# iosefa/obia

Measured on AMD Instinct MI355X. Metric: Mpixel/s (SLIC+zonal feats) on 16384²×8-band; achieved HBM GB/s fraction, higher is better.
Workload: dtype f32

## Files before the change

obia_amd/csrc/slic_spatial.hip:

```cpp

#ifdef OBIA_RUN_STATS
__device__ unsigned long long g_run_stats[16];
#define RS_DECL unsigned long long rs_t = clock64(); unsigned rs_c[8] = {0, 0, 0, 0, 0, 0, 0, 0};
#define RS_COUNT(i, v) rs_c[i] += (unsigned)(v);
#define RS_TICK(i) { const unsigned long long rs_n = clock64(); if ((threadIdx.x & 63) == 0) atomicAdd(&g_run_stats[i], rs_n - rs_t); rs_t = rs_n; }
#define RS_FLUSH { for (int rs_i = 1; rs_i < 8; ++rs_i) { unsigned rs_v = rs_c[rs_i]; for (int rs_o = 32; rs_o; rs_o >>= 1) rs_v += __shfl_xor(rs_v, rs_o); \
                   if ((threadIdx.x & 63) == 0) atomicAdd(&g_run_stats[rs_i], (unsigned long long)rs_v); } if ((threadIdx.x & 63) == 0) atomicAdd(&g_run_stats[0], 1ull); }
extern "C" void obia_debug_run_stats(unsigned long long *out, int reset) {
    (void)hipMemcpyFromSymbol(out, HIP_SYMBOL(g_run_stats), sizeof(unsigned long long) * 16);
    if (reset) { unsigned long long z[16] = {0}; (void)hipMemcpyToSymbol(HIP_SYMBOL(g_run_stats), z, sizeof(z)); }
}
#else
#define RS_DECL
#define RS_COUNT(i, v)
#define RS_TICK(i)
#define RS_FLUSH
#endif

constexpr float RUN_REL = 0x1p-19f, RUN_ABS = 0x1p-60f, RUN_W_LO = 0x1p-30f, RUN_W_HI = 0x1p90f;

template <int CP>
__device__ __forceinline__ void slic_spatial_tile(const SlicProblem &P, int gtile, int tile, int l_n, const unsigned *__restrict__ mask4,
                                                  const float *__restrict__ cent, unsigned long long *__restrict__ acc, int RQ,
                                                  unsigned long long *__restrict__ px_counter, int *__restrict__ orphan_flag,
                                                  const int *__restrict__ tl_k, const unsigned *__restrict__ tl_fp) {
    constexpr int RS = CENT_REC + CP;
    constexpr int NW = NT / 64;
    constexpr unsigned INF_BITS = 0x7f800000u;
    __shared__ __attribute__((aligned(16))) float r_hdr[MAXC][CENT_REC];
    __shared__ int r_k[MAXC];
    __shared__ unsigned long long r_acc[MAXC];
    __shared__ unsigned char r_surv[NW][SWEEP_TW / FB][64];
    __shared__ unsigned r_q[NW][128];

    const int tid = threadIdx.x;
    const int wv = __builtin_amdgcn_readfirstlane(tid >> 6);
    const int ty0 = (tile / P.tiles_x) * SWEEP_TH, tx0 = (tile % P.tiles_x) * SWEEP_TW;
    const float w = P.spatial_w;
    RS_DECL
    if (px_counter && tile == 0 && tid == 0) atomicAdd(px_counter, (unsigned long long)P.H * (unsigned long long)P.W);

    int lk = -1;
    if (tid < l_n) lk = tl_k[(size_t)gtile * MAXC + tid];
    const unsigned myc4 = tl_fp[(size_t)gtile * NT + tid];
    if (tid < MAXC) r_acc[tid] = 0ull;
    if (lk >= 0) {
        const float4 *src = reinterpret_cast<const float4 *>(cent + (size_t)lk * RS);
        const float4 a = src[0], b = src[1];
        float4 *dh = reinterpret_cast<float4 *>(&r_hdr[tid][0]);
        dh[0] = a; dh[1] = b;
        r_k[tid] = lk;
    }
    const int nc = l_n;
    __syncthreads();
    RS_TICK(8)

    const int fy0 = ty0 + FB * wv;
    if (fy0 < P.H) {
        const int fy1 = min(fy0 + FB, P.H);
        const int lane = lane_now();
        int cnt[SWEEP_TW / FB];
#pragma unroll
        for (int bxi = 0; bxi < SWEEP_TW / FB; ++bxi) {
            const int fx0 = tx0 + FB * bxi;
            cnt[bxi] = 0;
            if (fx0 >= P.W) continue;
            const int fx1 = min(fx0 + FB, P.W);
            const unsigned c = (myc4 >> (8 * bxi)) & 0xffu;
            unsigned lbb = 0xffffffffu, ubb = INF_BITS;
            bool hit = false;
            if (c != 0xffu) {
                const float4 h0 = *reinterpret_cast<const float4 *>(&r_hdr[c][0]);
                const float2 h1 = *reinterpret_cast<const float2 *>(&r_hdr[c][4]);
                const int y0 = __float_as_int(h0.z), y1 = __float_as_int(h0.w), x0 = __float_as_int(h1.x), x1 = __float_as_int(h1.y);
                if (y0 < fy1 && y1 > fy0 && x0 < fx1 && x1 > fx0) {
                    hit = true;
                    const float cy = h0.x, cx = h0.y;
                    const float ylo = (float)fy0, yhi = (float)(fy1 - 1), xlo = (float)fx0, xhi = (float)(fx1 - 1);
                    const float ry = (cy < ylo) ? ylo : ((cy > yhi) ? yhi : cy), rx = (cx < xlo) ? xlo : ((cx > xhi) ? xhi : cx);
                    const float tyn = cy - ry, txn = cx - rx;
                    lbb = __float_as_uint((tyn * tyn + txn * txn) * w);
                    if (y0 <= fy0 && y1 >= fy1 && x0 <= fx0 && x1 >= fx1) {
                        const float tyf = fmaxf(fabsf(cy - ylo), fabsf(cy - yhi)), txf = fmaxf(fabsf(cx - xlo), fabsf(cx - xhi));
                        ubb = __float_as_uint((tyf * tyf + txf * txf) * w);
                    }
                }
            }
            const unsigned bound = wave_umin(ubb);
            bool surv = hit && lbb <= bound;
            if (bound != INF_BITS) {
                const int la = (int)__builtin_ctzll(__ballot(ubb == bound));
                const int ca = __builtin_amdgcn_readlane((int)c, la);
                const float4 ha = *reinterpret_cast<const float4 *>(&r_hdr[ca][0]);
                const float4 hb = *reinterpret_cast<const float4 *>(&r_hdr[surv ? c : ca][0]);
                const float ylo = (float)fy0, yhi = (float)(fy1 - 1), xlo = (float)fx0, xhi = (float)(fx1 - 1);
                const float ay0 = (ha.x - ylo) * (ha.x - ylo), ay1 = (ha.x - yhi) * (ha.x - yhi), ax0 = (ha.y - xlo) * (ha.y - xlo), ax1 = (ha.y - xhi) * (ha.y - xhi);
                const float by0 = (hb.x - ylo) * (hb.x - ylo), by1 = (hb.x - yhi) * (hb.x - yhi), bx0 = (hb.y - xlo) * (hb.y - xlo), bx1 = (hb.y - xhi) * (hb.y - xhi);
                const float a00 = (ay0 + ax0) * w, a01 = (ay0 + ax1) * w, a10 = (ay1 + ax0) * w, a11 = (ay1 + ax1) * w;
                const float g = fminf(fminf((by0 + bx0) * w - a00, (by0 + bx1) * w - a01), fminf((by1 + bx0) * w - a10, (by1 + bx1) * w - a11));
                const float M = fmaxf(fmaxf(a00, a01), fmaxf(a10, a11));
                if (M < 3.0e38f && g > RUN_REL * M + RUN_ABS * w) surv = false;
            }
            const unsigned long long m = __ballot(surv);
            const unsigned pos = __builtin_amdgcn_mbcnt_hi((unsigned)(m >> 32), __builtin_amdgcn_mbcnt_lo((unsigned)m, 0u));
            if (surv) r_surv[wv][bxi][pos] = (unsigned char)c;
            cnt[bxi] = __popcll(m);
        }
        wave_lds_sync();
        RS_TICK(9)

        const int seg = lane >> 4, y = fy0 + (lane & 15), xa = tx0 + FB * seg;
        const int mycnt = seg == 0 ? cnt[0] : (seg == 1 ? cnt[1] : (seg == 2 ? cnt[2] : cnt[3]));
        const unsigned char *sv = &r_surv[wv][seg][0];
        unsigned rowbits = 0u;
        if (y < P.H && xa < P.W) {
            const int n = min(FB, P.W - xa);
            if ((long long)P.n_valid == (long long)P.H * (long long)P.W) {
                rowbits = 0xffffu >> (FB - n);
            } else {
                const unsigned *mp = mask4 + ((long long)P.m4_off + (long long)(y >> 2) * P.W + xa);
                const int sh = 8 * (y & 3);
#pragma unroll
                for (int i = 0; i < FB; ++i) {
                    const unsigned v = (i < n) ? mp[i] : 0u;
                    rowbits |= (unsigned)(((v >> sh) & 0xffu) != 0u) << i;
                }
            }
        }
        const float fy = (float)y;
        bool orphan = false;
        auto add_run = [&](int k, int a, int b) {
            const unsigned bits = rowbits & (0xffffu >> (FB - 1 - (b - xa))) & (0xffffu << (a - xa)) & 0xffffu;
            if (!bits) return;
            if (k < 0) { orphan = true; return; }
            const unsigned m = __popc(bits);
            const unsigned sx = __popc(bits & 0xaaaau) + 2u * __popc(bits & 0xccccu) + 4u * __popc(bits & 0xf0f0u) + 8u * __popc(bits & 0xff00u) +
                                m * (unsigned)(xa - tx0);
// ... 47 lines not shown
                int m = xl + (int)(gl / (gl + gr) * (float)(len - 1));
                m = max(xl + 1, min(m, xr - 2));
                const int p0 = m - 1, p3 = m + 2;
                const float fp0 = (float)p0, fm = (float)m, fm1 = (float)(m + 1), fp3 = (float)p3;
                float e1p0 = INFINITY, e2p0 = INFINITY, e1p3 = INFINITY, e2p3 = INFINITY, e1m = INFINITY, e1m1 = INFINITY, dump = INFINITY;
                int kp0 = -1, kp3 = -1, km = -1, km1 = -1;
                for (int i = 0; i < mycnt; ++i) {
                    const int c = sv[i];
                    const float4 h0 = *reinterpret_cast<const float4 *>(&r_hdr[c][0]);
                    const float2 h1 = *reinterpret_cast<const float2 *>(&r_hdr[c][4]);
                    const int y0 = __float_as_int(h0.z), y1 = __float_as_int(h0.w), x0 = __float_as_int(h1.x), x1 = __float_as_int(h1.y);
                    if ((unsigned)(y - y0) >= (unsigned)(y1 - y0)) continue;
                    const float ty = h0.x - fy, dy2 = ty * ty;
                    const float t0 = h0.y - fp0, t1 = h0.y - fm, t2 = h0.y - fm1, t3 = h0.y - fp3;
                    take((dy2 + t0 * t0) * w, p0 >= x0 && p0 < x1, c, e1p0, e2p0, kp0);
                    take((dy2 + t1 * t1) * w, m >= x0 && m < x1, c, e1m, dump, km);
                    take((dy2 + t2 * t2) * w, m + 1 >= x0 && m + 1 < x1, c, e1m1, dump, km1);
                    take((dy2 + t3 * t3) * w, p3 >= x0 && p3 < x1, c, e1p3, e2p3, kp3);
                }
                const bool okl = kp0 == k1l && (p0 == xl || margin(d1l, d2l, e1p0, e2p0));
                const bool okr = kp3 == k1r && (p3 == xr || margin(e1p3, e2p3, d1r, d2r));
                bool mdone = false, m1done = false;
                if (okl) { mdone = km == k1l; add_run(k1l, xl, mdone ? m : p0); } else q0 = entry(xl, p0);
                if (okr) { m1done = km1 == k1r; add_run(k1r, m1done ? m + 1 : p3, xr); } else q1 = entry(p3, xr);
                if (!mdone) add_run(km, m, m);
                if (!m1done) add_run(km1, m + 1, m + 1);
            } else {
                q0 = entry(xl, xr);
            }
        }
        int qn = 0;
        {
            const unsigned long long m0 = __ballot(q0 != 0xffffffffu);
            if (q0 != 0xffffffffu) r_q[wv][__builtin_amdgcn_mbcnt_hi((unsigned)(m0 >> 32), __builtin_amdgcn_mbcnt_lo((unsigned)m0, 0u))] = q0;
            qn = __popcll(m0);
            const unsigned long long m1 = __ballot(q1 != 0xffffffffu);
            if (q1 != 0xffffffffu) r_q[wv][qn + __builtin_amdgcn_mbcnt_hi((unsigned)(m1 >> 32), __builtin_amdgcn_mbcnt_lo((unsigned)m1, 0u))] = q1;
            qn += __popcll(m1);
        }
        wave_lds_sync();
        RS_TICK(10)
        RS_COUNT(5, lane == 0 ? qn : 0)
        for (int base = 0; base < qn; base += 4) {
            const int ei = base + (lane >> 4);
            if (ei >= qn) continue;
            const unsigned e = r_q[wv][ei];
            const int xrel = (int)(e & 15u) + (lane & 15);
            if (xrel > (int)((e >> 4) & 15u) || !((e >> (16 + xrel)) & 1u)) continue;
            RS_COUNT(6, 1)
            const int qs = (int)((e >> 12) & 3u), qy = fy0 + (int)((e >> 8) & 15u), qx = tx0 + FB * qs + xrel;
            const int qcnt = qs == 0 ? cnt[0] : (qs == 1 ? cnt[1] : (qs == 2 ? cnt[2] : cnt[3]));
            const unsigned char *qv = &r_surv[wv][qs][0];
            const float fqy = (float)qy, fqx = (float)qx;
            float best = INFINITY;
            int bk = -1;
            for (int i = 0; i < qcnt; ++i) {
                const int c = qv[i];
                const float4 h0 = *reinterpret_cast<const float4 *>(&r_hdr[c][0]);
                const float2 h1 = *reinterpret_cast<const float2 *>(&r_hdr[c][4]);
                const int y0 = __float_as_int(h0.z), y1 = __float_as_int(h0.w), x0 = __float_as_int(h1.x), x1 = __float_as_int(h1.y);
                if (!(qy >= y0 && qy < y1 && qx >= x0 && qx < x1)) continue;
                const float ty = h0.x - fqy, tx = h0.y - fqx;
                const float d = (ty * ty + tx * tx) * w;
                if (d < best) { best = d; bk = c; }
            }
            if (bk < 0) orphan = true;
            else atomicAdd(&r_acc[bk], 1ull | ((unsigned long long)(unsigned)(qy - ty0) << 16) | ((unsigned long long)(unsigned)(qx - tx0) << 40));
        }
        if (__ballot(orphan) && lane == 0) *orphan_flag = 1;
        RS_TICK(11)
        RS_FLUSH
    }
    __syncthreads();
    const int tid_e = wv * 64 + lane_now();
    for (int i = tid_e; i < nc * 3; i += NT) {
        const int slot = i / 3, q = i - slot * 3;
        const unsigned long long pw = r_acc[slot];
        const unsigned long long n = pw & 0xffffull;
        if (n == 0ull) continue;
        const unsigned long long v = q == 0 ? n : (q == 1 ? ((pw >> 16) & 0xffffffull) + n * (unsigned long long)ty0 : (pw >> 40) + n * (unsigned long long)tx0);
        atomicAdd(&acc[(size_t)r_k[slot] * RQ + CP + q], v);
    }
    RS_TICK(12)
}

template <int CP>
__global__ __launch_bounds__(NT) __attribute__((amdgpu_waves_per_eu(LEAN_WAVES, LEAN_WAVES))) void slic_spatial_kernel(OBIA_ASSIGN_PARAMS) {
    constexpr int XG = OBIA_XCD_GROUP;
    const int gtile = tile_base + (((int)(blockIdx.x >> 3) / XG) * 8 + (int)(blockIdx.x & 7)) * XG + (int)(blockIdx.x >> 3) % XG;
    if (gtile >= total_tiles_all) return;
    const int l_n = tl_meta[2 * (size_t)gtile], l_bw = tl_meta[2 * (size_t)gtile + 1], l_req = tl_req[gtile];
    const int prob_i = tiles_per_prob > 0 ? gtile / tiles_per_prob : tile_prob[gtile];
    const SlicProblem P = probs[prob_i];
    const bool listed = l_n >= 0 && l_bw >= 0 && l_req <= (l_bw & 0xffff);
    if (listed && accumulate && !store_labels && !P.direct && P.spatial_w >= RUN_W_LO && P.spatial_w <= RUN_W_HI)
        slic_spatial_tile<CP>(P, gtile, gtile - P.tile_off, l_n, mask4, cent, acc, RQ, px_counter, orphan_flag, tl_k, tl_fp);
    else
        slic_assign_body<CP, true, true, false, false, true, false>(OBIA_ASSIGN_ARGS);
}
```

obia_amd/csrc/slic_sweep.hip:

```cpp
#include "slic.hpp"

#include <type_traits>
#include <hip/hip_ext.h>

#include <cstdlib>

namespace obia {

#ifdef OBIA_STAMP
__device__ unsigned long long g_tl[65536 * 4 * 24];
#define STAMP_DECL unsigned long long st_t = clock64(), st_t0 = st_t, st_r0 = __builtin_amdgcn_s_memrealtime(), st_acc[12] = {0, 0, 0, 0, 0, 0, 0, 0, 0, 0, 0, 0}, st_cnt[6] = {0, 0, 0, 0, 0, 0};
#define STAMP_COUNT(i, v) st_cnt[i] += (v);
#define STAMP(i) { const unsigned long long st_n = clock64(); st_acc[i] += st_n - st_t; st_t = st_n; }
#ifndef OBIA_STAMP_KIND
#define OBIA_STAMP_KIND 0
#endif
#define STAMP_FLUSH if (accumulate && (LEAN ? 1 : 0) == OBIA_STAMP_KIND && (threadIdx.x & 63) == 0 && gtile < 65536) { unsigned long long *st_o = g_tl + ((size_t)gtile * 4 + (threadIdx.x >> 6)) * 24; for (int st_i = 0; st_i < 12; ++st_i) st_o[st_i] = st_acc[st_i]; st_o[12] = st_t0; st_o[13] = clock64(); st_o[14] = st_r0; st_o[15] = __builtin_amdgcn_s_memrealtime(); for (int st_i = 0; st_i < 6; ++st_i) st_o[16 + st_i] = st_cnt[st_i]; }
#else
#define STAMP_DECL
#define STAMP(i)
#define STAMP_COUNT(i, v)
#define STAMP_FLUSH
#endif

// ... 240 lines not shown

__device__ __forceinline__ void wave_lds_sync() {
    asm volatile("" ::: "memory");
    __builtin_amdgcn_wave_barrier();
    asm volatile("" ::: "memory");
}

__device__ __forceinline__ int lane_now() { return (int)__builtin_amdgcn_mbcnt_hi(~0u, __builtin_amdgcn_mbcnt_lo(~0u, 0u)); }

template <int CP>
__device__ __forceinline__ void global_accumulate(unsigned long long *__restrict__ acc, int RQ, int k, unsigned y, unsigned x,
                                                  const float *f, float fs) {
    unsigned long long *a = acc + (size_t)k * RQ;
#pragma unroll
    for (int ch = 0; ch < CP; ++ch) atomicAdd(&a[ch], (unsigned long long)(long long)to_fixed32(f[ch], fs));
    atomicAdd(&a[CP], 1ull);
    atomicAdd(&a[CP + 1], (unsigned long long)y);
    atomicAdd(&a[CP + 2], (unsigned long long)x);
}

__device__ __forceinline__ bool orphan_needs_repeat(int store_labels, int sweep_id) {
    return store_labels == 0 || (store_labels == 1 && sweep_id > 1);
}

template <int CP, bool MASKED, bool IGNORE_COLOR, bool SLICZERO>
__device__ void slow_tile(const SlicProblem &P, int ty0, int tx0, const float *__restrict__ feat,
                          const uint8_t *__restrict__ mask, const float *__restrict__ cent,
                          const int *__restrict__ head, int32_t *__restrict__ labels,
                          unsigned long long *__restrict__ acc, int RQ, int accumulate, int accum_color, int start_label,
                          float fs, int store_labels, int *__restrict__ orphan_flag, int sweep_id, int nch) {
    constexpr int RS = CENT_REC + CP;
    const float w = P.spatial_w;
    for (int i = threadIdx.x; i < SWEEP_TW * SWEEP_TH; i += NT) {
        const int y = ty0 + i / SWEEP_TW, x = tx0 + i % SWEEP_TW;
        if (y >= P.H || x >= P.W) continue;
        const long long pix = P.pix_off + (long long)y * P.W + x;
        if (MASKED && mask[pix] == 0) { labels[pix] = start_label - 1; continue; }
        float f[CP];
#pragma unroll
        for (int ch = 0; ch < CP; ++ch) f[ch] = ch < nch ? feat_at(feat, P, CP, y, x, ch) : 0.0f;
        int by_lo = (y - 2 * P.sy - 2) / P.sy; if (y - 2 * P.sy - 2 < 0) by_lo = 0;
        int by_hi = (y + 2 * P.sy + 2) / P.sy; if (by_hi > P.ncy - 1) by_hi = P.ncy - 1;
        int bx_lo = (x - 2 * P.sx - 2) / P.sx; if (x - 2 * P.sx - 2 < 0) bx_lo = 0;
        int bx_hi = (x + 2 * P.sx + 2) / P.sx; if (bx_hi > P.ncx - 1) bx_hi = P.ncx - 1;
        float best = INFINITY;
        int bk = -1;
        for (int by = by_lo; by <= by_hi; ++by)
            for (int bx = bx_lo; bx <= bx_hi; ++bx)
                for (int cur = head[P.cell_off + by * P.ncx + bx]; cur >= 0; cur = reinterpret_cast<const int *>(cent + (size_t)cur * RS)[6]) {
                    const float *rec = cent + (size_t)cur * RS;
                    const int *irec = reinterpret_cast<const int *>(rec);
                    if (!(y >= irec[2] && y < irec[3] && x >= irec[4] && x < irec[5])) continue;
                    const float tyv = P.sp_y * (rec[0] - (float)y), txv = P.sp_x * (rec[1] - (float)x);
                    const float dy2 = tyv * tyv, dx2 = txv * txv;
                    float d = (dy2 + dx2) * w;
                    if (!IGNORE_COLOR) {
                        float dc = 0.0f;
#pragma unroll
                        for (int ch = 0; ch < CP; ++ch) { const float t = f[ch] - rec[CENT_REC + ch]; dc += t * t; }
                        d += SLICZERO ? dc / rec[7] : dc;
                    }
                    if (d < best || (d == best && cur < bk)) { best = d; bk = cur; }
                }
        int k = bk;
        if (k < 0) {
            if (orphan_needs_repeat(store_labels, sweep_id)) *orphan_flag = 1;
            if (store_labels == 2) {
                const int prev = labels[pix];
                if (prev >= start_label) k = prev - start_label + P.cent_off;
            }
        } else {
            labels[pix] = k - P.cent_off + start_label;
        }
        if (accumulate && k >= 0) {
            if (!accum_color) {
#pragma unroll
                for (int ch = 0; ch < CP; ++ch) f[ch] = 0.0f;
            }
            global_accumulate<CP>(acc, RQ, k, (unsigned)y, (unsigned)x, f, fs);
        }
    }
}

template <int CP, bool MASKED, bool IGNORE_COLOR, bool FIXPT, bool SLICZERO, bool LEAN, bool COLLB, int NCH = CP>
__device__ __forceinline__ void slic_assign_body(
    const SlicProblem *__restrict__ probs, const float *__restrict__ feat, const uint8_t *__restrict__ mask,
    const unsigned *__restrict__ mask4, const float *__restrict__ cent, const int *__restrict__ head,
    int32_t *__restrict__ labels, unsigned long long *__restrict__ acc, int RQ, int accumulate, int store_labels,
    int start_label, float fs, const int *__restrict__ bin_stamp, int *__restrict__ tile_lp,
    int *__restrict__ cache_k, unsigned long long *__restrict__ cache_q, int sweep_id, int use_cache,
    unsigned long long *__restrict__ px_counter, const int *__restrict__ tile_prob, int total_tiles_all,
    int *__restrict__ orphan_flag, int tiles_per_prob, const float *__restrict__ fbox, int tile_base, int nch_arg,
    int *__restrict__ tl_k, unsigned *__restrict__ tl_fp, int *__restrict__ tl_meta, const int *__restrict__ tl_req) {
    const int nch_rt = (NCH < CP) ? NCH : nch_arg;
    constexpr int accum_color = LEAN ? 0 : 1;
#ifdef OBIA_ABL_NOACC
    accumulate = 0;
#endif
#ifndef OBIA_XCD_GROUP
#define OBIA_XCD_GROUP 2
#endif
    constexpr int XG = OBIA_XCD_GROUP;
    const int gtile = tile_base + (((int)(blockIdx.x >> 3) / XG) * 8 + (int)(blockIdx.x & 7)) * XG + (int)(blockIdx.x >> 3) % XG;
    if (gtile >= total_tiles_all) return;
    const int l_n = tl_meta[2 * (size_t)gtile], l_bw = tl_meta[2 * (size_t)gtile + 1], l_req = tl_req[gtile];
    const int l_built = l_bw < 0 ? -1 : (l_bw & 0xffff), l_streak = l_bw < 0 ? 0 : (l_bw >> 16);
    STAMP_DECL
    constexpr int RS = CENT_REC + CP;
    const int prob_i = tiles_per_prob > 0 ? gtile / tiles_per_prob : tile_prob[gtile];
    const SlicProblem P = probs[prob_i];
    const int tile = gtile - P.tile_off;
    constexpr int AQ = LEAN ? 1 : CP + 1;
    constexpr int PWI = LEAN ? 0 : CP;
    constexpr int NPASS = (CP + 7) / 8;

    __shared__ __attribute__((aligned(16))) float s_hdr[MAXC][CENT_REC];
    __shared__ __attribute__((aligned(16))) float s_col[COLLB ? MAXC : 1][COLLB ? CP : 4];
    __shared__ __attribute__((aligned(16))) int s_k[MAXC];
    __shared__ unsigned char s_fls[NT / 64][64];
    __shared__ unsigned long long s_acc[MAXC][AQ];
    constexpr int NF = LEAN ? 1 : CP + 1;
#ifndef OBIA_FOLD_LAYERS
#define OBIA_FOLD_LAYERS 1
#endif
    constexpr int FOLD_LAYERS = LEAN ? 0 : OBIA_FOLD_LAYERS;
    constexpr int FLD = FOLD_LAYERS > 0 ? FOLD_LAYERS : 1;
    __shared__ int s_tf[LEAN ? 1 : NT / 64][FLD][NF][LEAN ? 1 : 65];
    __shared__ int s_tkey[LEAN ? 1 : NT / 64][FLD][LEAN ? 1 : 64];
    __shared__ unsigned s_orph[SWEEP_TH * SWEEP_TW / 32];
    __shared__ int s_cnt, s_uncacheable;
#ifdef OBIA_ABL_LDSPAD
    __shared__ int s_pad[OBIA_ABL_LDSPAD / 4];
    if (start_label == 12345) s_pad[threadIdx.x] = 1;
#endif

    const int tid = threadIdx.x, lane = tid & 63;
    const int wv = __builtin_amdgcn_readfirstlane(tid >> 6);
    const int ty0 = (tile / P.tiles_x) * SWEEP_TH, tx0 = (tile % P.tiles_x) * SWEEP_TW;
    const int ty1 = min(ty0 + SWEEP_TH, P.H), tx1 = min(tx0 + SWEEP_TW, P.W);
    if (P.direct) {
        slow_tile<CP, MASKED, IGNORE_COLOR, SLICZERO>(P, ty0, tx0, feat, mask, cent, head, labels, acc, RQ, accumulate,
                                                      accum_color, start_label, fs, store_labels, orphan_flag, sweep_id, nch_rt);
        return;
    }

    const float w = P.spatial_w;
    const int fy0 = ty0 + FB * wv;
    const int fy0_o = fy0;
    const bool wave_active = fy0 < P.H;
    const int fy1 = min(fy0 + FB, P.H);
    const int fy1_o = fy1;
    const bool want_feat = !IGNORE_COLOR || accum_color;
    v2f f2[LEAN ? 1 : CP][PPT / 2];
    unsigned mbw;
    const bool all_valid = (long long)P.n_valid == (long long)P.H * (long long)P.W;
    auto fetch = [&](int fx0, int yb, int lane_o, bool real) {
#ifdef OBIA_ABL_NOLOAD
        real = false;
#endif
        const int xx = fx0 + (lane_o & 15);
        if (MASKED && !all_valid) {
            const unsigned *mbase = mask4 + ((long long)P.m4_off + (long long)(fy0 >> 2) * P.W + fx0);
            const unsigned moff = (real && (yb < P.H) && (xx < P.W)) ? (unsigned)(lane_o >> 4) * (unsigned)P.W + (unsigned)(lane_o & 15) : 0u;
            mbw = mbase[moff];
        } else {
            mbw = 0x01010101u;
        }
        if (!LEAN && want_feat) {
            const float4 *pb = reinterpret_cast<const float4 *>(feat) +
                               (P.feat_off + ((long long)(fy0 >> 2) * P.XB + (fx0 >> 4)) * ((LEAN ? 0 : CP) * 16));
            const unsigned fob = (real && (yb < P.H) && (xx < P.W))
                                     ? ((unsigned)(lane_o >> 4) * (unsigned)((LEAN ? 0 : CP) * 16 * P.XB) + (unsigned)(lane_o & 15)) * 16u : 0u;
#pragma unroll
            for (int ch = 0; ch < (LEAN ? 1 : CP); ++ch) {
                if (ch >= nch_rt) { f2[ch][0] = splat(0.0f); f2[ch][1] = splat(0.0f); continue; }
                const float4 t = ld_stream_f4(reinterpret_cast<const char *>(pb + ch * 16) + (size_t)fob);
                f2[ch][0] = (v2f){t.x, t.y};
                f2[ch][1] = (v2f){t.z, t.w};
            }
        } else {
#pragma unroll
            for (int ch = 0; ch < (LEAN ? 1 : CP); ++ch) { f2[ch][0] = splat(0.0f); f2[ch][1] = splat(0.0f); }
        }
    };
    auto fetch_first = [&]() {
        const int lane_i = lane_now();
        fetch(tx0, fy0 + PPT * (lane_i >> 4), lane_i, true);
    };
    constexpr int GQ = CP + 3;
    const int tile_id = P.tile_off + tile;
    int by_lo = (ty0 - 2 * P.sy - 2) / P.sy; if (ty0 - 2 * P.sy - 2 < 0) by_lo = 0;
    int by_hi = (ty1 + 2 * P.sy + 1) / P.sy; if (by_hi > P.ncy - 1) by_hi = P.ncy - 1;
    int bx_lo = (tx0 - 2 * P.sx - 2) / P.sx; if (tx0 - 2 * P.sx - 2 < 0) bx_lo = 0;
    int bx_hi = (tx1 + 2 * P.sx + 1) / P.sx; if (bx_hi > P.ncx - 1) bx_hi = P.ncx - 1;
    const int nbw = bx_hi - bx_lo + 1;
    const int nbins = (by_hi - by_lo + 1) * nbw;
    if (FIXPT) {
        const int lp = use_cache ? tile_lp[tile_id] : 0;
        int dirty = lp <= 0;
        if (!dirty)
            for (int bi = tid; bi < nbins; bi += NT)
                dirty |= bin_stamp[P.cell_off + (by_lo + bi / nbw) * P.ncx + bx_lo + bi % nbw] > lp;
        if (!__syncthreads_or(dirty)) {
            if (accumulate) {
                const int *ck = cache_k + (size_t)tile_id * (MAXC + 1);
                const unsigned long long *cq = cache_q + (size_t)tile_id * MAXC * GQ;
                const int ne = ck[0];
                for (int i = tid; i < ne * GQ; i += NT) {
                    const int e = i / GQ, q = i - e * GQ;
                    const int k = ck[1 + e];
                    if (k < 0 || (q < CP && !accum_color)) continue;
                    atomicAdd(&acc[(size_t)k * RQ + q], cq[(size_t)e * GQ + q]);
                }
            }
            return;
        }
        if (px_counter && tid == 0) atomicAdd(&px_counter[tile & 255], (unsigned long long)(ty1 - ty0) * (unsigned long long)(tx1 - tx0));
    } else if (px_counter && tile == 0 && tid == 0) {
        atomicAdd(px_counter, (unsigned long long)P.H * (unsigned long long)P.W);
    }
#ifdef OBIA_NO_LISTS
    constexpr bool USE_LISTS = false;
#else
    constexpr bool USE_LISTS = !COLLB;
#endif
    const bool listed = USE_LISTS && l_n >= 0 && l_req <= l_built;
    unsigned myc4 = 0xffffffffu;
    auto clear_tables = [&]() {
        for (int i = tid; i < MAXC * AQ; i += NT) (&s_acc[0][0])[i] = 0ull;
        for (int i = tid; i < SWEEP_TH * SWEEP_TW / 32; i += NT) s_orph[i] = 0u;
        if (tid == 0) s_uncacheable = 0;
    };
    float4 r0 = make_float4(0.f, 0.f, 0.f, 0.f), r1 = r0, rcol[CP / 4];
#pragma unroll
    for (int q = 0; q < CP / 4; ++q) rcol[q] = r0;
    int nxt = -1;
    auto load_node = [&](int c) {
        const float4 *src = reinterpret_cast<const float4 *>(cent + (size_t)c * RS);
        r0 = src[0]; r1 = src[1];
        if (COLLB) {
#pragma unroll
            for (int q = 0; q < CP / 4; ++q) rcol[q] = src[2 + q];
        }
        nxt = __float_as_int(r1.z);
    };
    auto put_slot = [&](int slot, int k) {
        float4 *dh = reinterpret_cast<float4 *>(&s_hdr[slot][0]);
        dh[0] = r0; dh[1] = make_float4(r1.x, r1.y, __int_as_float(k), r1.w);
        s_k[slot] = k;
        if (COLLB) {
#pragma unroll
            for (int q = 0; q < CP / 4; ++q) *reinterpret_cast<float4 *>(&s_col[slot][4 * q]) = rcol[q];
        }
    };
    int nc;
    if (listed) {
        int lk = -1;
        if (tid < l_n) lk = tl_k[(size_t)gtile * MAXC + tid];
        myc4 = tl_fp[(size_t)gtile * NT + tid];
        clear_tables();
        if (lk >= 0) load_node(lk);
        if (wave_active) fetch_first();
        if (lk >= 0) put_slot(tid, lk);
        nc = l_n;
        __syncthreads();
        STAMP(1)
    } else {
        clear_tables();
        const int streak = (l_n >= 0 && sweep_id - l_built <= 1) ? l_streak + 1 : 0;
        int g = (!USE_LISTS || l_n == -2 || streak >= LIST_GIVE_UP || sweep_id >= 0xffff) ? 0 : LIST_G2;
        bool listable = g > 0;
        for (;;) {
            __syncthreads();
            if (tid < MAXC) s_k[tid] = 0x7fffffff;
            if (tid == 0) s_cnt = 0;
            __syncthreads();
            int gy_lo = (ty0 - 2 * P.sy - 2 - g) / P.sy; if (ty0 - 2 * P.sy - 2 - g < 0) gy_lo = 0;
            int gy_hi = (ty1 + 2 * P.sy + 1 + g) / P.sy; if (gy_hi > P.ncy - 1) gy_hi = P.ncy - 1;
            int gx_lo = (tx0 - 2 * P.sx - 2 - g) / P.sx; if (tx0 - 2 * P.sx - 2 - g < 0) gx_lo = 0;
            int gx_hi = (tx1 + 2 * P.sx + 1 + g) / P.sx; if (gx_hi > P.ncx - 1) gx_hi = P.ncx - 1;
            const int gbw = gx_hi - gx_lo + 1;
            const int gbins = (gy_hi - gy_lo + 1) * gbw;
            for (int bi = tid; bi < gbins; bi += NT) {
                int cur = head[P.cell_off + (gy_lo + bi / gbw) * P.ncx + gx_lo + bi % gbw];
                if (cur >= 0) load_node(cur);
                while (cur >= 0) {
                    const int y0 = __float_as_int(r0.z), y1 = __float_as_int(r0.w);
                    const int x0 = __float_as_int(r1.x), x1 = __float_as_int(r1.y);
                    if (y0 - g < ty1 && y1 + g > ty0 && x0 - g < tx1 && x1 + g > tx0) {
                        const int slot = atomicAdd(&s_cnt, 1);
                        if (slot < MAXC) put_slot(slot, cur);
                    }
                    cur = nxt;
                    if (cur >= 0) load_node(cur);
                }
            }
            __syncthreads();
            nc = s_cnt;
            if (nc > MAXC) {
                if (g > 0) { g = 0; listable = false; continue; }
                if (tid == 0) { tl_meta[2 * (size_t)gtile] = -2; tl_meta[2 * (size_t)gtile + 1] = sweep_id & 0xffff; }
                slow_tile<CP, MASKED, IGNORE_COLOR, SLICZERO>(P, ty0, tx0, feat, mask, cent, head, labels, acc, RQ, accumulate,
                                                              accum_color, start_label, fs, store_labels, orphan_flag, sweep_id, nch_rt);
                return;
            }
            {
                int myk = 0, rk = 0;
                if (tid < nc) {
                    myk = s_k[tid];
#pragma unroll 1
                    for (int i = 0; i < nc; i += 8) {
                        const int4 ka = *reinterpret_cast<const int4 *>(&s_k[i]), kb = *reinterpret_cast<const int4 *>(&s_k[i + 4]);
                        rk += (ka.x < myk) + (ka.y < myk) + (ka.z < myk) + (ka.w < myk) + (kb.x < myk) + (kb.y < myk) + (kb.z < myk) + (kb.w < myk);
                    }
                    r0 = *reinterpret_cast<const float4 *>(&s_hdr[tid][0]);
                    r1 = *reinterpret_cast<const float4 *>(&s_hdr[tid][4]);
                    if (COLLB) {
#pragma unroll
                        for (int q = 0; q < CP / 4; ++q) rcol[q] = *reinterpret_cast<const float4 *>(&s_col[tid][4 * q]);
                    }
                }
                __syncthreads();
                if (tid < nc) put_slot(rk, myk);
                __syncthreads();
            }
            bool ovf = false;
            myc4 = (nc <= 64 && lane < nc) ? (unsigned)lane * 0x01010101u : 0xffffffffu;
            for (int bxi = 0; nc > 64 && wave_active && bxi < SWEEP_TW / FB; ++bxi) {
                const int fx0 = tx0 + FB * bxi;
                if (fx0 >= P.W) break;
                const int fx1 = min(fx0 + FB, P.W);
                int base = 0;
                for (int r = 0; r < (MAXC + 63) / 64; ++r) {
                    const int c = 64 * r + lane;
                    bool in = false;
                    if (c < nc) {
                        const float4 h0 = *reinterpret_cast<const float4 *>(&s_hdr[c][0]);
                        const float4 h1 = *reinterpret_cast<const float4 *>(&s_hdr[c][4]);
                        in = (__float_as_int(h0.z) - g < fy1) && (__float_as_int(h0.w) + g > fy0) &&
                             (__float_as_int(h1.x) - g < fx1) && (__float_as_int(h1.y) + g > fx0);
                    }
                    const unsigned long long m = __ballot(in);
                    const int pos = base + __popcll(m & ((1ull << lane) - 1ull));
                    if (in && pos < 64) s_fls[wv][pos] = (unsigned char)c;
                    base += __popcll(m);
                }
                ovf |= base > 64;
                wave_lds_sync();
                const unsigned mine = (lane < base) ? (unsigned)s_fls[wv][lane] : 0xffu;
                myc4 = (myc4 & ~(0xffu << (8 * bxi))) | (mine << (8 * bxi));
                wave_lds_sync();
            }
            if (__syncthreads_or(ovf ? 1 : 0)) {
                if (g > 0) { g = 0; listable = false; continue; }
                if (tid == 0) { tl_meta[2 * (size_t)gtile] = -2; tl_meta[2 * (size_t)gtile + 1] = sweep_id & 0xffff; }
                slow_tile<CP, MASKED, IGNORE_COLOR, SLICZERO>(P, ty0, tx0, feat, mask, cent, head, labels, acc, RQ, accumulate,
                                                              accum_color, start_label, fs, store_labels, orphan_flag, sweep_id, nch_rt);
                return;
            }
            break;
        }
        if (listable) {
            if (tid < nc) tl_k[(size_t)gtile * MAXC + tid] = s_k[tid];
            tl_fp[(size_t)gtile * NT + tid] = myc4;
        }
        if (tid == 0) { tl_meta[2 * (size_t)gtile] = listable ? nc : -2; tl_meta[2 * (size_t)gtile + 1] = (sweep_id & 0xffff) | (streak << 16); }
        if (wave_active) fetch_first();
        STAMP(1)
    }
    STAMP(0)

    constexpr unsigned INF_BITS = 0x7f800000u;
    for (int bxi = 0; wave_active && bxi < SWEEP_TW / FB; ++bxi) {
        const int fx0 = tx0 + FB * bxi;
        if (fx0 >= P.W) break;
        const int lane_i = lane_now();
        const int yb_i = fy0 + PPT * (lane_i >> 4);
        const unsigned lrow_i = (unsigned)(PPT * (lane_i >> 4)) * (unsigned)P.W + (unsigned)(lane_i & 15);
        const int fx1 = min(fx0 + FB, P.W);
        const int x = fx0 + (lane_i & 15);
        const float fx = (float)x;
        unsigned long long bk[PPT];
#pragma unroll
        for (int j = 0; j < PPT; ++j) bk[j] = (unsigned long long)INF_BITS << 32;
#define BK_D(j) __uint_as_float((unsigned)(bk[j] >> 32))

        unsigned key = 0xffffffffu;
        int kkv = 0;
        float clbv = 0.0f;
        float blo[COLLB ? CP : 1], bhi[COLLB ? CP : 1];
        if (COLLB) {
            const float4 *bx = reinterpret_cast<const float4 *>(fbox) + (P.fb_off + (long long)(fy0_o >> 4) * P.XB + (fx0 >> 4)) * (2 * CP / 4);
#pragma unroll
            for (int q = 0; q < CP / 4; ++q) {
                const float4 l = bx[q], h = bx[CP / 4 + q];
                blo[4 * q] = l.x; blo[4 * q + 1] = l.y; blo[4 * q + 2] = l.z; blo[4 * q + 3] = l.w;
                bhi[4 * q] = h.x; bhi[4 * q + 1] = h.y; bhi[4 * q + 2] = h.z; bhi[4 * q + 3] = h.w;
            }
        }
        {
            const unsigned c = (myc4 >> (8 * bxi)) & 0xffu;
            int fy0 = fy0_o, fy1 = fy1_o;
            asm volatile("" : "+s"(fy0), "+s"(fy1));
            if (c != 0xffu) {
                const float4 h0 = *reinterpret_cast<const float4 *>(&s_hdr[c][0]);
                const float4 h1 = *reinterpret_cast<const float4 *>(&s_hdr[c][4]);
                kkv = __float_as_int(h1.z);
                const int y0 = __float_as_int(h0.z), y1 = __float_as_int(h0.w);
                const int x0 = __float_as_int(h1.x), x1 = __float_as_int(h1.y);
                if (y0 < fy1 && y1 > fy0 && x0 < fx1 && x1 > fx0) {
                    const float cy = h0.x, cx = h0.y;
                    const float ry = (cy < (float)fy0) ? (float)fy0 : ((cy > (float)(fy1 - 1)) ? (float)(fy1 - 1) : cy);
                    const float rx = (cx < (float)fx0) ? (float)fx0 : ((cx > (float)(fx1 - 1)) ? (float)(fx1 - 1) : cx);
                    const float tyv = cy - ry, txv = cx - rx;
                    float lb = (tyv * tyv + txv * txv) * w;
                    if (COLLB) {
                        float cl = 0.0f;
#pragma unroll
                        for (int q = 0; q < CP / 4; ++q) {
                            const float4 cc = *reinterpret_cast<const float4 *>(&s_col[c][4 * q]);
                            const float cv[4] = {cc.x, cc.y, cc.z, cc.w};
#pragma unroll
                            for (int e = 0; e < 4; ++e) {
                                const float t = fmaxf(fmaxf(blo[4 * q + e] - cv[e], cv[e] - bhi[4 * q + e]), 0.0f);
                                cl += t * t;
                            }
                        }
                        clbv = cl;
                        lb += cl;
                    }
                    key = (__float_as_uint(lb) & ~127u) | c;
                }
            }
        }

        STAMP(2)
        STAMP_COUNT(0, 1)
        float mybest = fmaxf(fmaxf(BK_D(0), BK_D(1)), fmaxf(BK_D(2), BK_D(3)));
#ifdef OBIA_ABL_VISITS
        int abl_visits = 0;
#endif
        unsigned mn = wave_umin(key);
        bool firstv = true;
        for (;;) {
            if (mn == 0xffffffffu) break;
            if (!firstv && !__ballot(__uint_as_float(mn & ~127u) <= mybest)) break;
#ifdef OBIA_ABL_VISITS
            if (++abl_visits > OBIA_ABL_VISITS) break;
#endif
// ... 636 lines not shown
```

Before: 6756.

## Build candidate lists inside the spatial fast path instead of falling back

Moves the per-tile candidate-list build into a shared helper and calls it from the spatial-only tile kernel, so tiles without a valid cached list no longer drop into the general assign body. Before, unlisted tiles took the heavier assign path; now the spatial path builds lists itself in LISTS_ONLY mode and only falls back when the tile cannot be listed. It also extends the debug run stats per sweep. The risks are extra LDS aliasing (r_q reused as scratch) and slightly more code in the spatial kernel.

```diff
diff --git a/obia_amd/csrc/slic_spatial.hip b/obia_amd/csrc/slic_spatial.hip
--- a/obia_amd/csrc/slic_spatial.hip
+++ b/obia_amd/csrc/slic_spatial.hip
@@ -1,14 +1,14 @@
 
 #ifdef OBIA_RUN_STATS
-__device__ unsigned long long g_run_stats[16];
-#define RS_DECL unsigned long long rs_t = clock64(); unsigned rs_c[8] = {0, 0, 0, 0, 0, 0, 0, 0};
+__device__ unsigned long long g_run_stats[10][16];
+#define RS_DECL unsigned long long rs_t = clock64(); unsigned rs_c[8] = {0, 0, 0, 0, 0, 0, 0, 0}; unsigned long long *const rs_g = g_run_stats[min(max(sweep_id, 0), 9)];
 #define RS_COUNT(i, v) rs_c[i] += (unsigned)(v);
-#define RS_TICK(i) { const unsigned long long rs_n = clock64(); if ((threadIdx.x & 63) == 0) atomicAdd(&g_run_stats[i], rs_n - rs_t); rs_t = rs_n; }
+#define RS_TICK(i) { const unsigned long long rs_n = clock64(); if ((threadIdx.x & 63) == 0) atomicAdd(&rs_g[i], rs_n - rs_t); rs_t = rs_n; }
 #define RS_FLUSH { for (int rs_i = 1; rs_i < 8; ++rs_i) { unsigned rs_v = rs_c[rs_i]; for (int rs_o = 32; rs_o; rs_o >>= 1) rs_v += __shfl_xor(rs_v, rs_o); \
-                   if ((threadIdx.x & 63) == 0) atomicAdd(&g_run_stats[rs_i], (unsigned long long)rs_v); } if ((threadIdx.x & 63) == 0) atomicAdd(&g_run_stats[0], 1ull); }
+                   if ((threadIdx.x & 63) == 0) atomicAdd(&rs_g[rs_i], (unsigned long long)rs_v); } if ((threadIdx.x & 63) == 0) { atomicAdd(&rs_g[0], 1ull); if (build) atomicAdd(&rs_g[13], 1ull); } }
 extern "C" void obia_debug_run_stats(unsigned long long *out, int reset) {
-    (void)hipMemcpyFromSymbol(out, HIP_SYMBOL(g_run_stats), sizeof(unsigned long long) * 16);
-    if (reset) { unsigned long long z[16] = {0}; (void)hipMemcpyToSymbol(HIP_SYMBOL(g_run_stats), z, sizeof(z)); }
+    (void)hipMemcpyFromSymbol(out, HIP_SYMBOL(g_run_stats), sizeof(unsigned long long) * 160);
+    if (reset) { unsigned long long z[160] = {0}; (void)hipMemcpyToSymbol(HIP_SYMBOL(g_run_stats), z, sizeof(z)); }
 }
 #else
 #define RS_DECL
@@ -20,15 +20,16 @@
 constexpr float RUN_REL = 0x1p-19f, RUN_ABS = 0x1p-60f, RUN_W_LO = 0x1p-30f, RUN_W_HI = 0x1p90f;
 
 template <int CP>
-__device__ __forceinline__ void slic_spatial_tile(const SlicProblem &P, int gtile, int tile, int l_n, const unsigned *__restrict__ mask4,
-                                                  const float *__restrict__ cent, unsigned long long *__restrict__ acc, int RQ,
+__device__ __forceinline__ bool slic_spatial_tile(const SlicProblem &P, int gtile, int tile, bool build, int l_n, int l_bw, int sweep_id,
+                                                  const unsigned *__restrict__ mask4, const float *__restrict__ cent,
+                                                  const int *__restrict__ head, unsigned long long *__restrict__ acc, int RQ,
                                                   unsigned long long *__restrict__ px_counter, int *__restrict__ orphan_flag,
-                                                  const int *__restrict__ tl_k, const unsigned *__restrict__ tl_fp) {
+                                                  int *__restrict__ tl_k, unsigned *__restrict__ tl_fp, int *__restrict__ tl_meta) {
     constexpr int RS = CENT_REC + CP;
     constexpr int NW = NT / 64;
     constexpr unsigned INF_BITS = 0x7f800000u;
     __shared__ __attribute__((aligned(16))) float r_hdr[MAXC][CENT_REC];
-    __shared__ int r_k[MAXC];
+    __shared__ __attribute__((aligned(16))) int r_k[MAXC];
     __shared__ unsigned long long r_acc[MAXC];
     __shared__ unsigned char r_surv[NW][SWEEP_TW / FB][64];
     __shared__ unsigned r_q[NW][128];
@@ -38,21 +39,34 @@
     const int ty0 = (tile / P.tiles_x) * SWEEP_TH, tx0 = (tile % P.tiles_x) * SWEEP_TW;
     const float w = P.spatial_w;
     RS_DECL
+
+    int nc;
+    unsigned myc4;
+    if (tid < MAXC) r_acc[tid] = 0ull;
+    if (build) {
+        const int fy0b = ty0 + FB * wv;
+        const int l_built = l_bw < 0 ? -1 : (l_bw & 0xffff), l_streak = l_bw < 0 ? 0 : (l_bw >> 16);
+        float (*no_col)[4] = nullptr;
+        if (slic_tile_build<CP, false, true, true>(P, gtile, ty0, min(ty0 + SWEEP_TH, P.H), tx0, min(tx0 + SWEEP_TW, P.W), fy0b, min(fy0b + FB, P.H),
+                                                   fy0b < P.H, cent, head, l_n, l_built, l_streak, sweep_id, r_hdr, no_col, r_k,
+                                                   reinterpret_cast<unsigned char (*)[64]>(&r_q[0][0]), reinterpret_cast<int *>(&r_q[NW - 1][64]),
+                                                   tl_k, tl_fp, tl_meta, nc, myc4) != BUILD_OK)
+            return false;
+    } else {
+        int lk = -1;
+        if (tid < l_n) lk = tl_k[(size_t)gtile * MAXC + tid];
+        myc4 = tl_fp[(size_t)gtile * NT + tid];
+        if (lk >= 0) {
+            const float4 *src = reinterpret_cast<const float4 *>(cent + (size_t)lk * RS);
+            const float4 a = src[0], b = src[1];
+            float4 *dh = reinterpret_cast<float4 *>(&r_hdr[tid][0]);
+            dh[0] = a; dh[1] = b;
+            r_k[tid] = lk;
+        }
+        nc = l_n;
+        __syncthreads();
+    }
     if (px_counter && tile == 0 && tid == 0) atomicAdd(px_counter, (unsigned long long)P.H * (unsigned long long)P.W);
-
-    int lk = -1;
-    if (tid < l_n) lk = tl_k[(size_t)gtile * MAXC + tid];
-    const unsigned myc4 = tl_fp[(size_t)gtile * NT + tid];
-    if (tid < MAXC) r_acc[tid] = 0ull;
-    if (lk >= 0) {
-        const float4 *src = reinterpret_cast<const float4 *>(cent + (size_t)lk * RS);
-        const float4 a = src[0], b = src[1];
-        float4 *dh = reinterpret_cast<float4 *>(&r_hdr[tid][0]);
-        dh[0] = a; dh[1] = b;
-        r_k[tid] = lk;
-    }
-    const int nc = l_n;
-    __syncthreads();
     RS_TICK(8)
 
     const int fy0 = ty0 + FB * wv;
@@ -266,6 +280,7 @@
         atomicAdd(&acc[(size_t)r_k[slot] * RQ + CP + q], v);
     }
     RS_TICK(12)
+    return true;
 }
 
 template <int CP>
@@ -277,8 +292,9 @@
     const int prob_i = tiles_per_prob > 0 ? gtile / tiles_per_prob : tile_prob[gtile];
     const SlicProblem P = probs[prob_i];
     const bool listed = l_n >= 0 && l_bw >= 0 && l_req <= (l_bw & 0xffff);
-    if (listed && accumulate && !store_labels && !P.direct && P.spatial_w >= RUN_W_LO && P.spatial_w <= RUN_W_HI)
-        slic_spatial_tile<CP>(P, gtile, gtile - P.tile_off, l_n, mask4, cent, acc, RQ, px_counter, orphan_flag, tl_k, tl_fp);
-    else
-        slic_assign_body<CP, true, true, false, false, true, false>(OBIA_ASSIGN_ARGS);
+    if (l_n != -2 && accumulate && !store_labels && !P.direct && P.spatial_w >= RUN_W_LO && P.spatial_w <= RUN_W_HI &&
+        slic_spatial_tile<CP>(P, gtile, gtile - P.tile_off, !listed, l_n, l_bw, sweep_id, mask4, cent, head, acc, RQ, px_counter, orphan_flag,
+                              tl_k, tl_fp, tl_meta))
+        return;
+    slic_assign_body<CP, true, true, false, false, true, false>(OBIA_ASSIGN_ARGS);
 }
diff --git a/obia_amd/csrc/slic_sweep.hip b/obia_amd/csrc/slic_sweep.hip
--- a/obia_amd/csrc/slic_sweep.hip
+++ b/obia_amd/csrc/slic_sweep.hip
@@ -346,6 +346,152 @@
     }
 }
 
+template <int CP, bool COLLB>
+struct StagedRecord {
+    float4 r0, r1, rcol[CP / 4];
+    int nxt;
+    __device__ __forceinline__ void clear() {
+        r0 = make_float4(0.f, 0.f, 0.f, 0.f); r1 = r0; nxt = -1;
+#pragma unroll
+        for (int q = 0; q < CP / 4; ++q) rcol[q] = r0;
+    }
+    __device__ __forceinline__ void load(const float *__restrict__ cent, int c) {
+        const float4 *src = reinterpret_cast<const float4 *>(cent + (size_t)c * (CENT_REC + CP));
+        r0 = src[0]; r1 = src[1];
+        if (COLLB) {
+#pragma unroll
+            for (int q = 0; q < CP / 4; ++q) rcol[q] = src[2 + q];
+        }
+        nxt = __float_as_int(r1.z);
+    }
+    __device__ __forceinline__ void put(float (*s_hdr)[CENT_REC], float (*s_col)[COLLB ? CP : 4], int *s_k, int slot, int k) const {
+        float4 *dh = reinterpret_cast<float4 *>(&s_hdr[slot][0]);
+        dh[0] = r0; dh[1] = make_float4(r1.x, r1.y, __int_as_float(k), r1.w);
+        s_k[slot] = k;
+        if (COLLB) {
+#pragma unroll
+            for (int q = 0; q < CP / 4; ++q) *reinterpret_cast<float4 *>(&s_col[slot][4 * q]) = rcol[q];
+        }
+    }
+};
+
+enum { BUILD_OK = 0, BUILD_SLOW = 1, BUILD_UNLISTABLE = 2 };
+template <int CP, bool COLLB, bool USE_LISTS, bool LISTS_ONLY>
+__device__ __forceinline__ int slic_tile_build(const SlicProblem &P, int gtile, int ty0, int ty1, int tx0, int tx1, int fy0, int fy1,
+                                               bool wave_active, const float *__restrict__ cent, const int *__restrict__ head,
+                                               int l_n, int l_built, int l_streak, int sweep_id,
+                                               float (*s_hdr)[CENT_REC], float (*s_col)[COLLB ? CP : 4], int *s_k,
+                                               unsigned char (*s_fls)[64], int *s_cnt,
+                                               int *__restrict__ tl_k, unsigned *__restrict__ tl_fp, int *__restrict__ tl_meta,
+                                               int &nc_out, unsigned &myc4_out) {
+    const int tid = threadIdx.x, lane = tid & 63;
+    const int wv = __builtin_amdgcn_readfirstlane(tid >> 6);
+    StagedRecord<CP, COLLB> rec;
+    rec.clear();
+    int nc;
+    unsigned myc4;
+    const int streak = (l_n >= 0 && sweep_id - l_built <= 1) ? l_streak + 1 : 0;
+    int g = (!USE_LISTS || l_n == -2 || streak >= LIST_GIVE_UP || sweep_id >= 0xffff) ? 0 : LIST_G2;
+    bool listable = g > 0;
+    if (LISTS_ONLY && !listable) return BUILD_UNLISTABLE;
+    for (;;) {
+        __syncthreads();
+        if (tid < MAXC) s_k[tid] = 0x7fffffff;
+        if (tid == 0) *s_cnt = 0;
+        __syncthreads();
+        int gy_lo = (ty0 - 2 * P.sy - 2 - g) / P.sy; if (ty0 - 2 * P.sy - 2 - g < 0) gy_lo = 0;
+        int gy_hi = (ty1 + 2 * P.sy + 1 + g) / P.sy; if (gy_hi > P.ncy - 1) gy_hi = P.ncy - 1;
+        int gx_lo = (tx0 - 2 * P.sx - 2 - g) / P.sx; if (tx0 - 2 * P.sx - 2 - g < 0) gx_lo = 0;
+        int gx_hi = (tx1 + 2 * P.sx + 1 + g) / P.sx; if (gx_hi > P.ncx - 1) gx_hi = P.ncx - 1;
+        const int gbw = gx_hi - gx_lo + 1;
+        const int gbins = (gy_hi - gy_lo + 1) * gbw;
+        for (int bi = tid; bi < gbins; bi += NT) {
+            int cur = head[P.cell_off + (gy_lo + bi / gbw) * P.ncx + gx_lo + bi % gbw];
+            if (cur >= 0) rec.load(cent, cur);
+            while (cur >= 0) {
+                const int y0 = __float_as_int(rec.r0.z), y1 = __float_as_int(rec.r0.w);
+                const int x0 = __float_as_int(rec.r1.x), x1 = __float_as_int(rec.r1.y);
+                if (y0 - g < ty1 && y1 + g > ty0 && x0 - g < tx1 && x1 + g > tx0) {
+                    const int slot = atomicAdd(s_cnt, 1);
+                    if (slot < MAXC) rec.put(s_hdr, s_col, s_k, slot, cur);
+                }
+                cur = rec.nxt;
+                if (cur >= 0) rec.load(cent, cur);
+            }
+        }
+        __syncthreads();
+        nc = *s_cnt;
+        if (nc > MAXC) {
+            if (LISTS_ONLY) return BUILD_UNLISTABLE;
+            if (g > 0) { g = 0; listable = false; continue; }
+            if (tid == 0) { tl_meta[2 * (size_t)gtile] = -2; tl_meta[2 * (size_t)gtile + 1] = sweep_id & 0xffff; }
+            return BUILD_SLOW;
+        }
+        {
+            int myk = 0, rk = 0;
+            if (tid < nc) {
+                myk = s_k[tid];
+#pragma unroll 1
+                for (int i = 0; i < nc; i += 8) {
+                    const int4 ka = *reinterpret_cast<const int4 *>(&s_k[i]), kb = *reinterpret_cast<const int4 *>(&s_k[i + 4]);
+                    rk += (ka.x < myk) + (ka.y < myk) + (ka.z < myk) + (ka.w < myk) + (kb.x < myk) + (kb.y < myk) + (kb.z < myk) + (kb.w < myk);
+                }
+                rec.r0 = *reinterpret_cast<const float4 *>(&s_hdr[tid][0]);
+                rec.r1 = *reinterpret_cast<const float4 *>(&s_hdr[tid][4]);
+                if (COLLB) {
+#pragma unroll
+                    for (int q = 0; q < CP / 4; ++q) rec.rcol[q] = *reinterpret_cast<const float4 *>(&s_col[tid][4 * q]);
+                }
+            }
+            __syncthreads();
+            if (tid < nc) rec.put(s_hdr, s_col, s_k, rk, myk);
+            __syncthreads();
+        }
+        bool ovf = false;
+        myc4 = (nc <= 64 && lane < nc) ? (unsigned)lane * 0x01010101u : 0xffffffffu;
+        for (int bxi = 0; nc > 64 && wave_active && bxi < SWEEP_TW / FB; ++bxi) {
+            const int fx0 = tx0 + FB * bxi;
+            if (fx0 >= P.W) break;
+            const int fx1 = min(fx0 + FB, P.W);
+            int base = 0;
+            for (int r = 0; r < (MAXC + 63) / 64; ++r) {
+                const int c = 64 * r + lane;
+                bool in = false;
+                if (c < nc) {
+                    const float4 h0 = *reinterpret_cast<const float4 *>(&s_hdr[c][0]);
+                    const float4 h1 = *reinterpret_cast<const float4 *>(&s_hdr[c][4]);
+                    in = (__float_as_int(h0.z) - g < fy1) && (__float_as_int(h0.w) + g > fy0) &&
+                         (__float_as_int(h1.x) - g < fx1) && (__float_as_int(h1.y) + g > fx0);
+                }
+                const unsigned long long m = __ballot(in);
+                const int pos = base + __popcll(m & ((1ull << lane) - 1ull));
+                if (in && pos < 64) s_fls[wv][pos] = (unsigned char)c;
+                base += __popcll(m);
+            }
+            ovf |= base > 64;
+            wave_lds_sync();
+            const unsigned mine = (lane < base) ? (unsigned)s_fls[wv][lane] : 0xffu;
+            myc4 = (myc4 & ~(0xffu << (8 * bxi))) | (mine << (8 * bxi));
+            wave_lds_sync();
+        }
+        if (__syncthreads_or(ovf ? 1 : 0)) {
+            if (LISTS_ONLY) return BUILD_UNLISTABLE;
+            if (g > 0) { g = 0; listable = false; continue; }
+            if (tid == 0) { tl_meta[2 * (size_t)gtile] = -2; tl_meta[2 * (size_t)gtile + 1] = sweep_id & 0xffff; }
+            return BUILD_SLOW;
+        }
+        break;
+    }
+    if (listable) {
+        if (tid < nc) tl_k[(size_t)gtile * MAXC + tid] = s_k[tid];
+        tl_fp[(size_t)gtile * NT + tid] = myc4;
+    }
+    if (tid == 0) { tl_meta[2 * (size_t)gtile] = listable ? nc : -2; tl_meta[2 * (size_t)gtile + 1] = (sweep_id & 0xffff) | (streak << 16); }
+    nc_out = nc;
+    myc4_out = myc4;
+    return BUILD_OK;
+}
+
 template <int CP, bool MASKED, bool IGNORE_COLOR, bool FIXPT, bool SLICZERO, bool LEAN, bool COLLB, int NCH = CP>
 __device__ __forceinline__ void slic_assign_body(
     const SlicProblem *__restrict__ probs, const float *__restrict__ feat, const uint8_t *__restrict__ mask,
@@ -495,140 +641,27 @@
         for (int i = tid; i < SWEEP_TH * SWEEP_TW / 32; i += NT) s_orph[i] = 0u;
         if (tid == 0) s_uncacheable = 0;
     };
-    float4 r0 = make_float4(0.f, 0.f, 0.f, 0.f), r1 = r0, rcol[CP / 4];
-#pragma unroll
-    for (int q = 0; q < CP / 4; ++q) rcol[q] = r0;
-    int nxt = -1;
-    auto load_node = [&](int c) {
-        const float4 *src = reinterpret_cast<const float4 *>(cent + (size_t)c * RS);
-        r0 = src[0]; r1 = src[1];
-        if (COLLB) {
-#pragma unroll
-            for (int q = 0; q < CP / 4; ++q) rcol[q] = src[2 + q];
-        }
-        nxt = __float_as_int(r1.z);
-    };
-    auto put_slot = [&](int slot, int k) {
-        float4 *dh = reinterpret_cast<float4 *>(&s_hdr[slot][0]);
-        dh[0] = r0; dh[1] = make_float4(r1.x, r1.y, __int_as_float(k), r1.w);
-        s_k[slot] = k;
-        if (COLLB) {
-#pragma unroll
-            for (int q = 0; q < CP / 4; ++q) *reinterpret_cast<float4 *>(&s_col[slot][4 * q]) = rcol[q];
-        }
-    };
     int nc;
     if (listed) {
+        StagedRecord<CP, COLLB> rec;
         int lk = -1;
         if (tid < l_n) lk = tl_k[(size_t)gtile * MAXC + tid];
         myc4 = tl_fp[(size_t)gtile * NT + tid];
         clear_tables();
-        if (lk >= 0) load_node(lk);
+        if (lk >= 0) rec.load(cent, lk);
         if (wave_active) fetch_first();
-        if (lk >= 0) put_slot(tid, lk);
+        if (lk >= 0) rec.put(s_hdr, s_col, s_k, tid, lk);
         nc = l_n;
         __syncthreads();
         STAMP(1)
     } else {
         clear_tables();
-        const int streak = (l_n >= 0 && sweep_id - l_built <= 1) ? l_streak + 1 : 0;
-        int g = (!USE_LISTS || l_n == -2 || streak >= LIST_GIVE_UP || sweep_id >= 0xffff) ? 0 : LIST_G2;
-        bool listable = g > 0;
-        for (;;) {
-            __syncthreads();
-            if (tid < MAXC) s_k[tid] = 0x7fffffff;
-            if (tid == 0) s_cnt = 0;
-            __syncthreads();
-            int gy_lo = (ty0 - 2 * P.sy - 2 - g) / P.sy; if (ty0 - 2 * P.sy - 2 - g < 0) gy_lo = 0;
-            int gy_hi = (ty1 + 2 * P.sy + 1 + g) / P.sy; if (gy_hi > P.ncy - 1) gy_hi = P.ncy - 1;
-            int gx_lo = (tx0 - 2 * P.sx - 2 - g) / P.sx; if (tx0 - 2 * P.sx - 2 - g < 0) gx_lo = 0;
-            int gx_hi = (tx1 + 2 * P.sx + 1 + g) / P.sx; if (gx_hi > P.ncx - 1) gx_hi = P.ncx - 1;
-            const int gbw = gx_hi - gx_lo + 1;
-            const int gbins = (gy_hi - gy_lo + 1) * gbw;
-            for (int bi = tid; bi < gbins; bi += NT) {
-                int cur = head[P.cell_off + (gy_lo + bi / gbw) * P.ncx + gx_lo + bi % gbw];
-                if (cur >= 0) load_node(cur);
-                while (cur >= 0) {
-                    const int y0 = __float_as_int(r0.z), y1 = __float_as_int(r0.w);
-                    const int x0 = __float_as_int(r1.x), x1 = __float_as_int(r1.y);
-                    if (y0 - g < ty1 && y1 + g > ty0 && x0 - g < tx1 && x1 + g > tx0) {
-                        const int slot = atomicAdd(&s_cnt, 1);
-                        if (slot < MAXC) put_slot(slot, cur);
-                    }
-                    cur = nxt;
-                    if (cur >= 0) load_node(cur);
-                }
-            }
-            __syncthreads();
-            nc = s_cnt;
-            if (nc > MAXC) {
-                if (g > 0) { g = 0; listable = false; continue; }
-                if (tid == 0) { tl_meta[2 * (size_t)gtile] = -2; tl_meta[2 * (size_t)gtile + 1] = sweep_id & 0xffff; }
-                slow_tile<CP, MASKED, IGNORE_COLOR, SLICZERO>(P, ty0, tx0, feat, mask, cent, head, labels, acc, RQ, accumulate,
-                                                              accum_color, start_label, fs, store_labels, orphan_flag, sweep_id, nch_rt);
-                return;
-            }
-            {
-                int myk = 0, rk = 0;
-                if (tid < nc) {
-                    myk = s_k[tid];
-#pragma unroll 1
-                    for (int i = 0; i < nc; i += 8) {
-                        const int4 ka = *reinterpret_cast<const int4 *>(&s_k[i]), kb = *reinterpret_cast<const int4 *>(&s_k[i + 4]);
-                        rk += (ka.x < myk) + (ka.y < myk) + (ka.z < myk) + (ka.w < myk) + (kb.x < myk) + (kb.y < myk) + (kb.z < myk) + (kb.w < myk);
-                    }
-                    r0 = *reinterpret_cast<const float4 *>(&s_hdr[tid][0]);
-                    r1 = *reinterpret_cast<const float4 *>(&s_hdr[tid][4]);
-                    if (COLLB) {
-#pragma unroll
-                        for (int q = 0; q < CP / 4; ++q) rcol[q] = *reinterpret_cast<const float4 *>(&s_col[tid][4 * q]);
-                    }
-                }
-                __syncthreads();
-                if (tid < nc) put_slot(rk, myk);
-                __syncthreads();
-            }
-            bool ovf = false;
-            myc4 = (nc <= 64 && lane < nc) ? (unsigned)lane * 0x01010101u : 0xffffffffu;
-            for (int bxi = 0; nc > 64 && wave_active && bxi < SWEEP_TW / FB; ++bxi) {
-                const int fx0 = tx0 + FB * bxi;
-                if (fx0 >= P.W) break;
-                const int fx1 = min(fx0 + FB, P.W);
-                int base = 0;
-                for (int r = 0; r < (MAXC + 63) / 64; ++r) {
-                    const int c = 64 * r + lane;
-                    bool in = false;
-                    if (c < nc) {
-                        const float4 h0 = *reinterpret_cast<const float4 *>(&s_hdr[c][0]);
-                        const float4 h1 = *reinterpret_cast<const float4 *>(&s_hdr[c][4]);
-                        in = (__float_as_int(h0.z) - g < fy1) && (__float_as_int(h0.w) + g > fy0) &&
-                             (__float_as_int(h1.x) - g < fx1) && (__float_as_int(h1.y) + g > fx0);
-                    }
-                    const unsigned long long m = __ballot(in);
-                    const int pos = base + __popcll(m & ((1ull << lane) - 1ull));
-                    if (in && pos < 64) s_fls[wv][pos] = (unsigned char)c;
-                    base += __popcll(m);
-                }
-                ovf |= base > 64;
-                wave_lds_sync();
-                const unsigned mine = (lane < base) ? (unsigned)s_fls[wv][lane] : 0xffu;
-                myc4 = (myc4 & ~(0xffu << (8 * bxi))) | (mine << (8 * bxi));
-                wave_lds_sync();
-            }
-            if (__syncthreads_or(ovf ? 1 : 0)) {
-                if (g > 0) { g = 0; listable = false; continue; }
-                if (tid == 0) { tl_meta[2 * (size_t)gtile] = -2; tl_meta[2 * (size_t)gtile + 1] = sweep_id & 0xffff; }
-                slow_tile<CP, MASKED, IGNORE_COLOR, SLICZERO>(P, ty0, tx0, feat, mask, cent, head, labels, acc, RQ, accumulate,
-                                                              accum_color, start_label, fs, store_labels, orphan_flag, sweep_id, nch_rt);
-                return;
-            }
-            break;
-        }
-        if (listable) {
-            if (tid < nc) tl_k[(size_t)gtile * MAXC + tid] = s_k[tid];
-            tl_fp[(size_t)gtile * NT + tid] = myc4;
-        }
-        if (tid == 0) { tl_meta[2 * (size_t)gtile] = listable ? nc : -2; tl_meta[2 * (size_t)gtile + 1] = (sweep_id & 0xffff) | (streak << 16); }
+        if (slic_tile_build<CP, COLLB, USE_LISTS, false>(P, gtile, ty0, ty1, tx0, tx1, fy0, fy1, wave_active, cent, head, l_n, l_built, l_streak,
+                                                         sweep_id, s_hdr, s_col, s_k, s_fls, &s_cnt, tl_k, tl_fp, tl_meta, nc, myc4) != BUILD_OK) {
+            slow_tile<CP, MASKED, IGNORE_COLOR, SLICZERO>(P, ty0, tx0, feat, mask, cent, head, labels, acc, RQ, accumulate,
+                                                          accum_color, start_label, fs, store_labels, orphan_flag, sweep_id, nch_rt);
+            return;
+        }
         if (wave_active) fetch_first();
         STAMP(1)
     }
```

Result: no change. 6694 (-0.9%).
